# purejade/pinot

Measured on AMD Instinct MI355X. Metric: rows/sec for filter+group-by SUM at 1/2/4/8 GPUs; % of HBM roofline, higher is better.
Workload: dtype int64; 1 GPU; c5: BASELINE configs[4]: 4096 x 2M rows sharded over the GPUs, (f1 IN 32 ids OR f2=7) AND f3<>3, group by gk (card 1000), sum(m); segments=4096, rows_total=8192000000, parallelism=dp1 (segment sharding)

## Files before the change

### pinot_amd/csrc/pgx_host.cpp

```cpp
#include "pgx_host.h"


namespace pgxh {
size_t align_up(size_t x, size_t a) { return (x + a - 1) & ~(a - 1); }

void canon_rprog(std::vector<int>& op, std::vector<int>& arg) {
  struct Node { int op, arg, l, r; };
  std::vector<Node> nodes;
  std::vector<int> st;
  for (size_t i = 0; i < op.size(); ++i) {
    Node nd{op[i], arg[i], -1, -1};
    if (op[i] == RP_NOT) {
      if (st.empty()) return;
      nd.l = st.back();
      st.pop_back();
    } else if (op[i] != RP_LEAF) {
      if (st.size() < 2) return;
      nd.r = st.back();
      st.pop_back();
      nd.l = st.back();
      st.pop_back();
    }
    nodes.push_back(nd);
    st.push_back(int(nodes.size()) - 1);
// ... 545 lines not shown
      J.narrow_vbits = P.part_narrow ? P.narrow_vd : 0;
      J.narrow_unit = P.kn.narrow_unit;
      J.prefetch2 = P.part_narrow && P.kn.prefetch2;
    }
    J.dense_slots = P.dense_slots;
    if ((K.group_mode == G_DENSE_LDS || K.group_mode == G_HASH64 || K.group_mode == G_HASH128) &&
        K.num_planes == 2 && K.num_aggs == 1 && (K.agg_kind[0] == A_SUM || K.agg_kind[0] == A_AVG) && !P.use_part) {
      const int c = K.agg_col[0];
      if (c >= 0 && J.cols[c].img != IMG_NONE && !J.cols[c].fp) {
        int64_t maxdocs = 1, ntiles = 0;
        uint64_t vrange = 0;
        const int64_t trows = int64_t(J.T) * J.TL;
        for (int sg : members) {
          maxdocs = std::max<int64_t>(maxdocs, P.ksegs[sg].num_docs);
          vrange = std::max<uint64_t>(vrange, P.segcols[sg][c]->vrange);
          ntiles += (int64_t(P.ksegs[sg].num_docs) + trows - 1) / trows;
        }
        maxdocs = std::min<int64_t>(maxdocs, (ntiles + cus - 1) / cus * trows);
        const int cb = bits_for(maxdocs + 1);
        const long double sum_max = (long double)maxdocs * (long double)(vrange + 1);
        int sb = 0;
        while (sb < 64 && std::ldexp(1.0L, sb) <= sum_max) ++sb;
        if (cb + sb <= 64) J.dense_pack = 64 - cb;
      }
    }
    if (hp1 && !J.dense_pack && hashg) {
      hp1 = false;
      while (hash_slots > 512 && lds_need() > lds_budget) hash_slots /= 2;
      J.hash_slots = hash_slots;
    }
    J.leafmask = P.fsm_on && P.lmask_off[members[0]] >= 0;
    J.compact = P.rchunk && !P.use_part;
    J.selmask = P.want_selmask;

    ExecPlan::JitGroup G;
    G.T = J.T;
    int lds_bytes = 0;
    std::string err;
    G.fn = jit_function(J, ctx->device, &lds_bytes, &err);
    if (!G.fn) fail(PGX_ERR_INTERNAL, "query kernel compile: " + err);
    const int64_t tile_rows = int64_t(J.T) * J.TL;
    int64_t tiles = 0;
    for (int s : members) {
      const KSeg& S = P.ksegs[s];
      JSeg js{};
      js.tile_begin = tiles;
      js.num_docs = S.num_docs;
      js.rec_base = P.rec_base[s];
      js.lmask = S.lmask;
      js.lmask_words = S.lmask_words;
      js.selmask = P.want_selmask ? P.sel_buf.as<unsigned int>() + P.sel_off[s] : nullptr;
      if (P.star[s].on) {
        auto& tl = P.star_tiles[s];
        tl.clear();
        for (const auto& r : P.star[s].ranges)
          for (int k = 0; k < r.second; ++k) {
            const int32_t a = P.blob32[r.first + 2 * k], b = P.blob32[r.first + 2 * k + 1];
            for (int64_t t = a / tile_rows; t <= b / tile_rows; ++t)
              if (tl.empty() || tl.back() != int32_t(t)) tl.push_back(int32_t(t));
          }
        std::sort(tl.begin(), tl.end());
        tl.erase(std::unique(tl.begin(), tl.end()), tl.end());
        const size_t off = star_tile_off;
        star_tile_off += tl.size();
        if (star_tile_off > P.star_tile_cap) fail(PGX_ERR_INTERNAL, "star tile list overflow");
        std::memcpy(B.host.bytes() + B.off_tiles + off * 4, tl.data(), tl.size() * 4);
// ... 1543 lines not shown
```

### pinot_amd/csrc/pgx_internal.h

```cpp
#pragma once
#include <stdint.h>

#include "pgx_jit_abi.h"

namespace pgx {

constexpr int kTileRows = 8192;
constexpr int kLaneRows = 32;
constexpr int kBlock = 256;
constexpr int kMaxQCols = 16;
constexpr int kMaxLeaves = 64;
constexpr int kInlineLeaves = PGX_J_MAX_LEAVES;
constexpr int kMaxLeafSlots = PGX_J_MAX_SLOTS;
constexpr int kStarMaxLeaves = 8;
constexpr int kMaxAggs = 8;
constexpr int kMaxGroupCols = 16;
constexpr int kMaxProg = 192;
constexpr int kStackDepth = 8;
constexpr uint64_t kEmptyKey = ~0ull;

enum LeafMode : int8_t {
  LEAF_SCAN_INTERVAL = 0,
  LEAF_SCAN_BITSET = 1,
  LEAF_RANGES = 2,
// ... 327 lines not shown
#include <vector>

namespace pgx {

enum ImgKind : int8_t {
  IMG_NONE = 0,
  IMG_U32 = 1,
  IMG_FOR16 = 2,
  IMG_F64 = 3,
};
constexpr int kImgFor16Blocks = 64;
constexpr int kLdsBudget = 160 * 1024 - 256;

constexpr uint64_t kNarrowC1 = 0x9E3779B1ull;
constexpr int kNarrow1Bits = 8;
constexpr int kNarrowRing = 64;
constexpr int kNarrowMaxBits2 = 10;
enum RProgKind { RPROG_AUTO = -1, RPROG_OFF = 0, RPROG_WAVE = 1, RPROG_SEG = 2, RPROG_CHUNK = 3, RPROG_STACK = 4 };
struct Knobs {
  bool jit = true;
  bool narrow = true;
  bool narrow_direct = false;
  bool narrow_gather = false;
  int rchunk = -1;
  int rprog = RPROG_AUTO;
  int batch_segs = -1;
  bool no_img = false;
  bool prefetch2 = false;
  int narrow_unit = 32;
  int lone_head = 2;
  bool part_small = false;
  int narrow_k2 = -1;
  bool narrow_log = false;
  bool host_profile = false;
};
Knobs read_knobs();

struct NarrowMix {
  uint64_t mask = 0, c1 = kNarrowC1, ic1 = 0;
  int s = 0;
};
inline uint64_t narrow_inverse(uint64_t c) {
  uint64_t x = c;
  for (int i = 0; i < 6; ++i) x *= 2 - c * x;
  return x;
}
inline NarrowMix narrow_mix(int keybits) {
  NarrowMix m;
  m.mask = keybits >= 64 ? ~0ull : (uint64_t(1) << keybits) - 1u;
  m.s = (keybits + 1) / 2;
  m.ic1 = narrow_inverse(m.c1);
  return m;
}

struct JitCol {
  int bits = 0;
  bool decode = false;
  int img = IMG_NONE;
  int img_sh = 0;
  int img_words = 0;
  bool acc32 = false;
  bool fp = false;
  bool remap = false;
  bool frac = false;
};

struct JitShape {
  int T = 256;
  int R = 8;
  int TL = 32;
  std::vector<JitCol> cols;
  std::vector<int> leaf_col, leaf_mode;
  std::vector<int> prog_op, prog_arg;
  std::vector<int> agg_kind, agg_col, plane_op;
  int group_mode = G_NONE;
  std::vector<int> gcol;
  std::vector<uint64_t> gmul;
  uint64_t dense_slots = 0;
  int num_planes = 1;
  std::vector<int> gshift;
  int keybits = 0;
  int emit_col = -1;
  std::vector<int> ghi;
  int hash_slots = 0;
  bool leafmask = false;
  std::vector<std::vector<int>> rprog_ops;
  int part_bits = 0;
  bool emit_dictid = false;
  bool part_slab = false;
  int dense_pack = 0;
  bool compact = false;
  bool selmask = false;
  bool part_narrow = false;
  int narrow_vbits = 0;
  int narrow_unit = 32;
  bool prefetch2 = false;
};

constexpr int kFsmMaxLeaves = 10;
constexpr int kFsmMaxStates = 4096;
constexpr uint64_t kFsmMaxTable = 1ull << 22;
constexpr int kFsmChunkRows = 1024;
constexpr int kFsmMaxIntervals = 3 * kFsmMaxLeaves + 2;

struct FsmTreeNode {
  int op = 0;
  int leaf = -1;
  int phys = 3;
  std::vector<FsmTreeNode> kids;
};
struct FsmSegInfo {
  int32_t num_docs = 0;
  std::vector<int64_t> sorted_first, sorted_last;
  uint32_t always_false = 0;
};
struct FsmPlan {
  int num_states = 0, num_leaves = 0, num_tables = 0;
  std::vector<uint32_t> table;
  std::vector<std::vector<std::pair<int32_t, int32_t>>> seg_intervals;
};
bool fsm_build(const FsmTreeNode& tree, int num_leaves, const std::vector<FsmSegInfo>& segs, FsmPlan& out,
               std::string* err);

std::string jit_source(const JitShape& s, int* lds_bytes);
void* jit_function(const JitShape& s, int device, int* lds_bytes, std::string* err);

}
```

### pinot_amd/csrc/pgx_jit.cpp

```cpp
#include <hip/hip_runtime.h>
#include <hip/hiprtc.h>
#include <sys/stat.h>
#include <unistd.h>

#include <algorithm>
#include <cstdio>
#include <cstdlib>
#include <map>
#include <mutex>
#include <sstream>
#include <string>
#include <vector>

#include "pgx_internal.h"

extern "C" int pgx_jit_compile_check(const char* source, char* log, unsigned long log_cap);

namespace pgx {

namespace {

const char* kAbiSrc =
#include "pgx_jit_abi.inc"
    ;
// ... 340 lines not shown
      }
    if (grouped)
      for (size_t g = 0; g < s.gcol.size(); ++g)
        if (s.cols[s.gcol[g]].remap) gremap[g] = split = true;
  }
  const bool pack = s.dense_pack > 0 && s.group_mode == G_DENSE_LDS && s.num_planes == 2 && naggs == 1 &&
                    (s.agg_kind[0] == A_SUM || s.agg_kind[0] == A_AVG) && !s.cols[s.agg_col[0]].fp &&
                    s.cols[s.agg_col[0]].img != IMG_NONE && !emit;
  for (int c = 0; c < ncols; ++c) {
    if (need_vb[c]) e.ln("const i64 vb", c, " = S->vbase[", c, "];");
    if (need_dict[c]) {
      if (s.cols[c].fp) e.ln("const PGX_G double* __restrict__ dd", c, " = (const PGX_G double*)S->dict[", c, "];");
      else e.ln("const PGX_G i64* __restrict__ di", c, " = (const PGX_G i64*)S->dict[", c, "];");
    }
  }
  if (scr_off >= 0) e.ln("int rc_cur = -1;  // chunk whose bitmap-program masks are in LDS");
  e.ln("u64 wcnt = 0;  // selected rows of this wave in this segment (wave-uniform)");
  if (!grouped) {
    for (int a = 0; a < naggs; ++a) {
      const int k = s.agg_kind[a];
      const int c = s.agg_col[a];
      if (k == A_SUM || k == A_AVG) {
        if (s.cols[c].fp) e.ln("double acc", a, " = 0.0;");
        else if (s.cols[c].img == IMG_NONE) e.ln("i64 acc", a, " = 0;");
        else e.ln("u64 acc", a, " = 0;");
      } else if (k == A_MIN) {
        e.ln("u32 mn", a, " = 0xFFFFFFFFu;");
      } else if (k == A_MAX) {
        e.ln("u32 mx", a, " = 0u;");
      }
    }
  }
  int gate = -1;
  {
    bool all_masks = !s.prog_op.empty();
    for (size_t pc = 0; pc < s.prog_op.size() && all_masks; ++pc)
      if (s.prog_op[pc] == OP_LEAF && !is_docmask(s.leaf_mode[s.prog_arg[pc]])) all_masks = false;
    std::vector<std::vector<int>> impl;
    for (size_t pc = 0; pc < s.prog_op.size() && all_masks; ++pc) {
      const int op = s.prog_op[pc], arg = s.prog_arg[pc];
      if (op == OP_LEAF) {
        impl.push_back(s.leaf_mode[arg] == LEAF_DOCMASK ? std::vector<int>{arg} : std::vector<int>{});
      } else if (op == OP_AND || op == OP_OR) {
        std::vector<int> acc = impl.back();
        impl.pop_back();
        for (int k = 1; k < arg; ++k) {
          std::vector<int> x = impl.back(), y;
          impl.pop_back();
          if (op == OP_AND) {
            y = acc;
            y.insert(y.end(), x.begin(), x.end());
          } else {
            for (int l : acc)
              if (std::find(x.begin(), x.end(), l) != x.end()) y.push_back(l);
          }
          acc = y;
        }
        impl.push_back(acc);
      } else if (op == OP_TRUE) {
        impl.push_back({});
      }
    }
    if (all_masks && impl.size() == 1 && !impl[0].empty() && !compact) gate = impl[0][0];
  }
  auto gate_bits = [&](const std::string& w) {
    return s.R == 32 ? w : "((" + w + " >> (r0 & 31)) & " + std::to_string((1u << s.R) - 1u) + "u)";
  };
  auto emit_loads = [&](const std::string& tile, const std::string& dst, const std::string& rbv = "rbn") {
    e.ln("{");
    e.ind++;
    e.ln(rbv, " = (int)((tl ? (long long)tl[", tile, " - tile0] : (", tile, " - tile0)) * (PT * PTL));");
    e.ln("const int rb = ", rbv, ";");
    e.ln("const bool full = rb + PT * PTL <= nd;");
    for (int u = 0; u < U; ++u) {
      e.ln("{");
      e.ind++;
      e.ln("const int r0 = rb + ", u * s.R, " * PT + tid * PR;");
      const std::string cond =
          gate >= 0 ? "(full || r0 < nd) && " + gate_bits("ga[" + std::to_string(u) + "]") + " != 0u" : "full || r0 < nd";
      for (int c = 0; c < ncols; ++c) {
        if (!s.cols[c].decode) continue;
        const int D = dwords_per(s, c);
        if (s.cols[c].frac)
          e.ln("if (", cond, ") pgx_ld_u<", D, ">(f", c, " + (((long long)r0 * ", s.cols[c].bits, ") >> 5), &", dst,
               c, "[", u * D, "]); else pgx_zero<", D, ">(&", dst, c, "[", u * D, "]);");
        else
        e.ln("if (", cond, ") pgx_ld<", D, ">(f", c, " + (long long)(r0 / PR) * ", D, ", &", dst, c, "[", u * D,
             "]); else pgx_zero<", D, ">(&", dst, c, "[", u * D, "]);");
      }
      for (int l = 0; l < nleaves; ++l)
        if (l == gate) e.ln(dst, "q", l, "[", u, "] = ga[", u, "];");
        else if (is_docmask(s.leaf_mode[l]))
          e.ln(dst, "q", l, "[", u, "] = (full || r0 < nd) ? dm", l, "[r0 >> 5] : 0u;");
      e.ind--;
      e.ln("}");
    }
// ... 100 lines not shown
        e.ln("    const u32 keep = dw >= nd ? 0u : (dw + 32 > nd ? (1u << (nd - dw)) - 1u : 0xFFFFFFFFu);");
      }
      std::vector<std::string> st;
      int leaf = 0, tmp = 0;
      for (int op : ops) {
        const std::string X = "y" + std::to_string(tmp++);
        if (op == RP_LEAF) {
          e.ln("    const u32 ", X, " = rlm", l, "[", leaf++ * 2048, " + w];");
        } else if (op == RP_NOT) {
          e.ln("    const u32 ", X, " = ~", st.back(), " & keep;");
          st.pop_back();
        } else {
          const std::string b = st.back();
          st.pop_back();
          const std::string a = st.back();
          st.pop_back();
          e.ln("    const u32 ", X, " = ", a, op == RP_AND ? " & " : " | ", b, ";");
        }
        st.push_back(X);
      }
      e.ln("    rlm", l, "[w] = ", st.empty() ? std::string("0u") : st.back(), ";");
      e.ln("  }");
    }
    e.ln("  pgx_lds_barrier();");
    e.ln("}");
  }
  e.ln("auto body = [&](auto FT) {");
  e.ind = 4;
  e.ln("constexpr bool FULL = decltype(FT)::value;");
  for (int u = 0; u < U; ++u) {
    e.ln("{");
    e.ind = 5;
    e.ln("const int r0 = rb + ", u * s.R, " * PT + tid * PR;");
    for (int c = 0; c < ncols; ++c) {
      if (!s.cols[c].decode) continue;
      e.ln("u32 v", c, "[PR];");
      if (s.cols[c].frac)
        e.ln("pgx_unpack_frac<", s.cols[c].bits, ", PR, ", dwords_per(s, c), ">(&c", c, "[", u * dwords_per(s, c),
             "], (u32)(((long long)r0 * ", s.cols[c].bits, ") & 31), v", c, ");");
      else
        e.ln("pgx_unpack<", s.cols[c].bits, ", PR>(&c", c, "[", u * dwords_per(s, c), "], v", c, ");");
    }
    for (int l = 0; l < nleaves; ++l) {
      if (s.leaf_mode[l] == LEAF_RANGES) e.ln("const u32 W", l, " = pgx_ranges_bits(rg", l, ", nr", l, ", cur", l, ", r0, PR);");
      if (is_docmask(s.leaf_mode[l])) e.ln("const u32 W", l, " = cq", l, "[", u, "] >> (r0 & 31);");
      if (s.leaf_mode[l] == LEAF_RCHUNK) e.ln("const u32 W", l, " = rlm", l, "[(r0 & 0xFFFF) >> 5] >> (r0 & 31);");
    }
    if (!grouped)
      for (int a = 0; a < naggs; ++a) {
        const int k = s.agg_kind[a];
        if ((k == A_SUM || k == A_AVG) && !s.cols[s.agg_col[a]].fp && s.cols[s.agg_col[a]].img != IMG_NONE &&
            s.cols[s.agg_col[a]].acc32)
          e.ln("u32 p", a, " = 0u;");
      }
    if (emit) e.ln("u64 recs[PR];");
    if (split) e.ln("u32 msk = 0u;");
    if (s.selmask) e.ln("u32 smk = 0u;");
    if (s.leafmask)
      for (int l = 0; l < nleaves; ++l) e.ln("u32 lw", l, " = 0u;");
    e.ln("#pragma unroll");
    e.ln("for (int j = 0; j < PR; ++j) {");
    e.ind = 6;
    e.ln("const bool vj = FULL || (r0 + j < nd);");
    std::vector<std::string> st;
    int tmp = 0;
    for (size_t pc = 0; pc < s.prog_op.size(); ++pc) {
      const int op = s.prog_op[pc], arg = s.prog_arg[pc];
      if (op == OP_LEAF) {
        const int l = arg, c = s.leaf_col[l];
        const std::string B = "b" + std::to_string(tmp++);
        const std::string v = "v" + std::to_string(c) + "[j]";
        switch (s.leaf_mode[l]) {
          case LEAF_SCAN_INTERVAL:
            e.ln("const bool ", B, " = vj && ((", v, " - lo", l, ") <= sp", l, ");");
            break;
          case LEAF_SCAN_BITSET:
            e.ln("const bool ", B, " = vj && ((bs", l, "[", v, " >> 5] >> (", v, " & 31u)) & 1u);");
            break;
          case LEAF_RANGES:
          case LEAF_DOCMASK:
          case LEAF_RCHUNK:
            e.ln("const bool ", B, " = vj && ((W", l, " >> j) & 1u);");
            break;
          case LEAF_DOCMASK_NOT:
            e.ln("const bool ", B, " = vj && !((W", l, " >> j) & 1u);");
            break;
          default:
// ... 155 lines not shown
          encs[a] = "ev" + std::to_string(a);
        }
      if (hpack) {
        const int c = s.agg_col[0];
        e.ln("const u64 hv = (1ull << ", s.dense_pack, ") + (u64)", img_value(s, c, img_off, "v" + std::to_string(c) + "[j]"),
             ";");
      }
      e.ln("const int ls = ", h128 ? "pgx_lhash128(hk, hst, " + std::to_string(HS) + ", klo, khi)"
                                   : "pgx_lhash64(hk, " + std::to_string(HS) + ", klo)", ";");
      e.ln("if (ls >= 0) {");
      if (hpack) {
        e.ln("  atomicAdd(&ht[ls], hv);");
      } else {
        e.ln("  atomicAdd(&ht[ls], 1ull);");
        for (int a = 0; a < naggs; ++a)
          if (s.agg_kind[a] != A_COUNT)
            e.ln("  ", plane_atomic(s.plane_op[a + 1], "&ht[" + std::to_string((a + 1) * HS) + " + ls]", encs[a]));
      }
      e.ln("} else {");
      e.ln("  const long long gs = ", h128 ? "pgx_ghash128((PGX_G unsigned long long*)A.hkeys, (PGX_G unsigned int*)A.hstate, A.hash_cap, klo, khi, A.overflow)"
                                           : "pgx_ghash64((PGX_G unsigned long long*)A.hkeys, A.hash_cap, klo, A.overflow)", ";");
      e.ln("  if (gs < 0) {");
      e.ln("    atomicAdd(A.overflow, 1ull);");
      e.ln("  } else {");
      e.ln("    atomicAdd(A.table + gs, 1ull);");
      for (int a = 0; a < naggs; ++a)
        if (s.agg_kind[a] != A_COUNT)
          e.ln("    ", plane_atomic(s.plane_op[a + 1], "A.table + " + std::to_string(a + 1) + " * A.hash_cap + gs", encs[a]));
      e.ln("  }");
      e.ln("}");
      e.ind = 6;
      e.ln("}");
    };
    if (!grouped) {
      for (int a = 0; a < naggs; ++a) {
        const int k = s.agg_kind[a];
        if (k == A_COUNT) continue;
        const int c = s.agg_col[a];
        const JitCol& C = s.cols[c];
        const std::string v = "v" + std::to_string(c) + "[j]";
        if (k == A_MIN) {
          e.ln("mn", a, " = min(mn", a, ", m ? ", v, " : 0xFFFFFFFFu);");
        } else if (k == A_MAX) {
          e.ln("mx", a, " = max(mx", a, ", m ? ", v, " : 0u);");
        } else if (C.fp) {
          const std::string val = (C.img == IMG_F64)
                                      ? "((const double*)lds)[" + std::to_string(img_off[c] / 8) + " + " + v + "]"
                                      : (gcolv[c] ? "gv" + std::to_string(c) + "[j]" : "dd" + std::to_string(c) + "[" + v + "]");
          e.ln("if (m) acc", a, " += ", val, ";");
        } else if (C.img == IMG_NONE) {
          if (gcolv[c]) e.ln("acc", a, " += gv", c, "[j];");
          else e.ln("if (m) acc", a, " += di", c, "[", v, "];");
        } else if (C.acc32) {
          e.ln("{ const u32 x = ", img_value(s, c, img_off, v), "; p", a, " += m ? x : 0u; }");
        } else {
          e.ln("{ const u32 x = ", img_value(s, c, img_off, v), "; acc", a, " += m ? (u64)x : 0ull; }");
        }
      }
    } else {
      if (emit) {
        e.ln("u64 rec = ~0ull;");
        e.ln("if (m) {");
        std::string key = "0ull";
        for (size_t g = 0; g < s.gcol.size(); ++g) {
          const int c = s.gcol[g];
          std::string id = "v" + std::to_string(c) + "[j]";
          if (s.cols[c].remap) id = "(u32)rm" + std::to_string(g) + "[" + id + "]";
          key += " | ((u64)" + id + " << " + std::to_string(s.gshift[g]) + ")";
        }
        std::string x = "0u";
        if (s.emit_col >= 0) {
          const std::string ec = std::to_string(s.emit_col);
          if (s.emit_dictid) x = "(u32)(v" + ec + "[j] + (u32)S->emit_rebase)";
          else x = s.cols[s.emit_col].img != IMG_NONE
                       ? "(u32)(" + img_value(s, s.emit_col, img_off, "v" + ec + "[j]") + " + (u32)S->emit_rebase)"
                       : "(u32)(di" + ec + "[v" + ec + "[j]] - S->vbase[" + ec + "] + S->emit_rebase)";
        }
        if (enarrow) {
          const NarrowMix mx = narrow_mix(s.keybits);
          const std::string M = std::to_string(mx.mask) + "ull";
          e.ln("  u64 h = ((", key, ") * ", mx.c1, "ull) & ", M, ";");
          e.ln("  h ^= h >> ", mx.s, ";");
          e.ln("  rec = ((h >> ", nrb1, ") << 56) | (h & ", (uint64_t(1) << nrb1) - 1u, "ull) | ((u64)(", x, ") << ", nrb1,
               ");");
        } else {
          e.ln("  rec = (", key, ") | ((u64)(", x, ") << ", s.keybits, ");");
        }
        e.ln("}");
        e.ln("recs[j] = rec;");
      } else if (hashm) {
        emit_hash();
      } else {
        emit_dense();
      }
    }
    e.ind = 5;
    e.ln("}");
    if (compact) {
      e.ln("  pgx_wave_lds_sync();");
      e.ln("}");
    }
    if (!grouped)
      for (int a = 0; a < naggs; ++a) {
        const int k = s.agg_kind[a];
        if ((k == A_SUM || k == A_AVG) && !s.cols[s.agg_col[a]].fp && s.cols[s.agg_col[a]].img != IMG_NONE &&
            s.cols[s.agg_col[a]].acc32)
          e.ln("acc", a, " += p", a, ";");
      }
    if (s.selmask) {
      const char* ty = s.R == 8 ? "unsigned char" : (s.R == 16 ? "unsigned short" : "unsigned int");
      e.ln("if (FULL || r0 < nd) ((PGX_G ", ty, "*)S->selmask)[r0 / PR] = (", ty, ")smk;");
    }
    if (s.leafmask) {
      const char* ty = s.R == 8 ? "unsigned char" : (s.R == 16 ? "unsigned short" : "unsigned int");
      e.ln("if (FULL || r0 < nd) {");
      for (int l = 0; l < nleaves; ++l)
        e.ln("  ((PGX_G ", ty, "*)(S->lmask + ", l, " * S->lmask_words))[r0 / PR] = (", ty, ")lw", l, ";");
      e.ln("}");
    }
    if (enarrow) {
      const std::string NR = std::to_string(NRG), NUs = std::to_string(NU);
      e.ln("{");
      e.ln("  u32 pp[PR];");
      e.ln("  #pragma unroll");
      e.ln("  for (int j = 0; j < PR; ++j) pp[j] = recs[j] != ~0ull ? atomicAdd(&ncur[(u32)(recs[j] >> 56)], 1u) : 0u;");
      e.ln("  pgx_lds_barrier();");
      e.ln("  const u32* const Ucur = nU + npar * 256;");
      e.ln("  const u32* const Vcur = nV + npar * 256;");
      e.ln("  if (tid < 256) {");
      e.ln("    const u32 en = ncur[tid], u0 = Ucur[tid], v0 = Vcur[tid];");
      e.ln("    const u32 lim = u0 + ", NR, "u;");
      e.ln("    const u32 nu = (((en < lim) ? en : lim) - u0) / ", NUs, "u;");
// ... 249 lines not shown
  int lds = 0;
};

std::mutex g_jit_mu;
std::map<std::pair<int, std::string>, JitEntry> g_jit_cache;

}

std::vector<int64_t> shape_key(const JitShape& s, int device) {
  std::vector<int64_t> k{device, s.T, s.R, s.TL, s.group_mode, int64_t(s.dense_slots), s.num_planes, s.keybits, s.emit_col,
                         int64_t(s.cols.size()), s.leafmask};
  for (const JitCol& c : s.cols)
    k.insert(k.end(), {c.bits, c.decode, c.img, c.img_sh, c.img_words, c.acc32, c.fp, c.remap, c.frac});
  auto add = [&](const auto& v) {
    k.push_back(-int64_t(v.size()) - 1);
    for (auto x : v) k.push_back(int64_t(x));
  };
  add(s.leaf_col);
  add(s.leaf_mode);
  add(s.prog_op);
  add(s.prog_arg);
  add(s.agg_kind);
  add(s.agg_col);
  add(s.plane_op);
  add(s.gcol);
  add(s.gmul);
  add(s.gshift);
  for (const auto& ops : s.rprog_ops) add(ops);
  k.push_back(s.part_bits);
  k.push_back(s.emit_dictid);
  k.push_back(s.part_slab);
  k.push_back(s.dense_pack);
  k.push_back(s.compact);
  k.push_back(s.selmask);
  k.push_back(s.part_narrow);
  k.push_back(s.narrow_vbits);
  k.push_back(s.narrow_unit);
  k.push_back(s.prefetch2);
  add(s.ghi);
  k.push_back(s.hash_slots);
  return k;
}

std::map<std::vector<int64_t>, JitEntry> g_jit_shapes;

constexpr const char* kJitOpts[] = {"--offload-arch=gfx950", "-O3", "-std=c++17"};

std::string jit_cache_dir() {
  const char* d = std::getenv("PGX_JIT_CACHE");
  return d && *d ? d : "";
}

uint64_t text_hash(const std::string& t, uint64_t h, uint64_t mul) {
  for (unsigned char c : t) {
    h ^= c;
    h *= mul;
  }
  return h;
}

std::string cache_text(const std::string& src) {
  std::string t = src;
  for (const char* o : kJitOpts) t += std::string("\n//") + o;
  return t;
}

// ... 77 lines not shown
      if (err) *err = "hiprtcCreateProgram failed";
      return nullptr;
    }
    const hiprtcResult rc = hiprtcCompileProgram(prog, 3, const_cast<const char**>(pgx::kJitOpts));
    if (rc != HIPRTC_SUCCESS) {
      size_t n = 0;
      hiprtcGetProgramLogSize(prog, &n);
      std::string log(n, '\0');
      if (n) hiprtcGetProgramLog(prog, &log[0]);
      hiprtcDestroyProgram(&prog);
      if (err) *err = "hiprtc compile failed: " + log.substr(0, 4000);
      return nullptr;
    }
    size_t code_size = 0;
    hiprtcGetCodeSize(prog, &code_size);
    code.assign(code_size, '\0');
    hiprtcGetCode(prog, &code[0]);
    hiprtcDestroyProgram(&prog);
    cache_store(src, code);
  }
  JitEntry ent;
  ent.lds = lds;
  if (hipModuleLoadData(&ent.mod, code.data()) != hipSuccess ||
      hipModuleGetFunction(&ent.fn, ent.mod, "pgxq") != hipSuccess) {
    if (err) *err = "hipModuleLoadData / hipModuleGetFunction failed";
    return nullptr;
  }
  g_jit_cache.emplace(key, ent);
  g_jit_shapes.emplace(skey, ent);
  return ent.fn;
}

}

extern "C" int pgx_jit_compile_check(const char* source, char* log, unsigned long log_cap) {
  hiprtcProgram prog;
  if (hiprtcCreateProgram(&prog, source, "pgx_query.hip", 0, nullptr, nullptr) != HIPRTC_SUCCESS) return -1;
  const hiprtcResult rc = hiprtcCompileProgram(prog, 3, const_cast<const char**>(pgx::kJitOpts));
  size_t n = 0;
  hiprtcGetProgramLogSize(prog, &n);
  if (log && log_cap) {
    std::string l(n, '\0');
    if (n) hiprtcGetProgramLog(prog, &l[0]);
    std::snprintf(log, log_cap, "%s", l.c_str());
  }
  if (rc == HIPRTC_SUCCESS)
    if (const char* dir = std::getenv("PGX_JIT_DUMP")) {
      size_t cs = 0;
      hiprtcGetCodeSize(prog, &cs);
      std::string code(cs, '\0');
      hiprtcGetCode(prog, &code[0]);
      if (FILE* f = std::fopen((std::string(dir) + "/last_check.co").c_str(), "wb")) {
        std::fwrite(code.data(), 1, cs, f);
        std::fclose(f);
      }
    }
  hiprtcDestroyProgram(&prog);
  return rc == HIPRTC_SUCCESS ? 0 : 1;
}

extern "C" int pgx_jit_selftest(int* n_total, char* log, unsigned long log_cap) {
  using namespace pgx;
  std::vector<JitShape> shapes;
  auto base = [](int bits_f, int bits_m, int img, int sh) {
    JitShape s;
    s.cols.resize(2);
// ... 125 lines not shown
    s.agg_col = {-1, 1, 1, 1, 1};
    s.plane_op = {P_ADD_I64, P_ADD_I64, P_ADD_I64, P_MIN_ORD, P_MAX_ORD, P_ADD_I64};
    s.num_planes = 6;
    shapes.push_back(s);
    s.cols[1].img = IMG_U32;
    s.cols[1].img_words = 1024;
    shapes.push_back(s);
    s.compact = false;
    s.selmask = true;
    shapes.push_back(s);
  }
  {
    JitShape s = base(10, 16, IMG_FOR16, 11);
    s.cols[1].img_words = 64 + 32768;
    s.cols.push_back(JitCol{});
    s.cols[2].bits = 10;
    s.cols[2].decode = false;
    s.leaf_col = {2, 2, 2, -1};
    s.leaf_mode = {LEAF_NONE, LEAF_NONE, LEAF_NONE, LEAF_DOCMASK};
    s.prog_op = {OP_LEAF, OP_STAT};
    s.prog_arg = {3, 0};
    s.R = 16;
    s.T = 1024;
    s.group_mode = G_DENSE_LDS;
    s.gcol = {0};
    s.gmul = {1};
    s.dense_slots = 1000;
    s.agg_kind = {A_SUM};
    s.agg_col = {1};
    s.plane_op = {P_ADD_I64, P_ADD_I64};
    s.num_planes = 2;
    s.dense_pack = 40;
    shapes.push_back(s);
  }
  for (int R : {8, 16, 32}) {
    JitShape s = base(R == 8 ? 8 : (R == 16 ? 10 : 7), 16, IMG_FOR16, 11);
    s.cols.push_back(JitCol{});
    s.cols[2].bits = 4;
    s.leaf_col = {0, 2, 0};
    s.leaf_mode = {LEAF_SCAN_INTERVAL, LEAF_RANGES, LEAF_DOCMASK_NOT};
    s.prog_op = {OP_LEAF, OP_LEAF, OP_LEAF, OP_OR, OP_AND};
    s.prog_arg = {0, 1, 2, 2, 2};
    s.R = R;
    s.leafmask = true;
    shapes.push_back(s);
  }
  {
    JitShape s = base(14, 16, IMG_FOR16, 11);
    s.cols.push_back(JitCol{});
    s.cols[2].bits = 20;
    s.cols[2].decode = true;
    s.leaf_col.clear();
    s.leaf_mode.clear();
    s.prog_op.clear();
    s.prog_arg.clear();
    s.R = 16;
    s.T = 512;
    s.group_mode = G_EMIT;
    s.gcol = {0, 2};
    s.gshift = {0, 14};
    s.keybits = 34;
    s.emit_col = 1;
    s.agg_kind = {A_SUM, A_MIN, A_MAX};
    s.agg_col = {1, 1, 1};
    s.plane_op = {P_ADD_I64, P_ADD_I64, P_MIN_ORD, P_MAX_ORD};
    s.num_planes = 4;
// ... 211 lines not shown
```

### pinot_amd/csrc/pgx_jit_device.h

```cpp
template <int D>
__device__ __forceinline__ void pgx_ld(const u32* __restrict__ gp, u32* w) {
  const PGX_G u32* p = (const PGX_G u32*)gp;
  if constexpr (D % 4 == 0) {
#pragma unroll
    for (int i = 0; i < D / 4; ++i) {
      pgx_u32x4 q = __builtin_nontemporal_load((const PGX_G pgx_u32x4*)p + i);
      w[4 * i] = q.x; w[4 * i + 1] = q.y; w[4 * i + 2] = q.z; w[4 * i + 3] = q.w;
    }
  } else if constexpr (D % 2 == 0) {
#pragma unroll
    for (int i = 0; i < D / 2; ++i) {
      pgx_u32x2 q = __builtin_nontemporal_load((const PGX_G pgx_u32x2*)p + i);
      w[2 * i] = q.x; w[2 * i + 1] = q.y;
    }
  } else {
#pragma unroll
    for (int i = 0; i < D; ++i) w[i] = __builtin_nontemporal_load(p + i);
  }
}

template <int D>
__device__ __forceinline__ void pgx_ld_u(const u32* __restrict__ gp, u32* w) {
  const PGX_G u32* p = (const PGX_G u32*)gp;
#pragma unroll
// ... 48 lines not shown
    for (int i = 0; i < D; ++i) w[i] = __builtin_bswap32(raw[i]);
    w[D] = 0u;
    constexpr u32 MASK = (1u << B) - 1u;
#pragma unroll
    for (int j = 0; j < R; ++j) {
      const int o = j * B;
      const int k = o >> 5;
      const int s = o & 31;
      if (s + B <= 32) v[j] = (w[k] >> (32 - s - B)) & MASK;
      else v[j] = __builtin_amdgcn_alignbit(w[k], w[k + 1], 64 - s - B) & MASK;
    }
  }
}

template <int B, int R, int DL>
__device__ __forceinline__ void pgx_unpack_frac(const u32* raw, u32 sh, u32* v) {
  u32 w[DL];
#pragma unroll
  for (int i = 0; i < DL; ++i) w[i] = __builtin_bswap32(raw[i]);
  constexpr int D = (R * B + 31) / 32;
  u32 x[D + 1];
#pragma unroll
  for (int i = 0; i < D; ++i) x[i] = sh ? __builtin_amdgcn_alignbit(w[i], i + 1 < DL ? w[i + 1] : 0u, 32u - sh) : w[i];
  x[D] = 0u;
  constexpr u32 MASK = (1u << B) - 1u;
#pragma unroll
  for (int j = 0; j < R; ++j) {
    const int o = j * B;
    const int k = o >> 5;
    const int s = o & 31;
    if (s + B <= 32) v[j] = (x[k] >> (32 - s - B)) & MASK;
    else v[j] = __builtin_amdgcn_alignbit(x[k], x[k + 1], 64 - s - B) & MASK;
  }
}

__device__ __forceinline__ u32 pgx_valid_bits(int r0, int nd, int R) {
  if (r0 >= nd) return 0u;
  const int n = nd - r0;
  if (n >= R) return (R == 32) ? 0xFFFFFFFFu : ((1u << R) - 1u);
  return (1u << n) - 1u;
}

__device__ __forceinline__ u32 pgx_ranges_bits(const PGX_G int* __restrict__ r, int nr, int& cur, int r0, int R) {
  while (cur < nr && r[2 * cur + 1] < r0) ++cur;
  u32 word = 0u;
  const int last = r0 + R - 1;
  for (int i = cur; i < nr; ++i) {
    const int a = r[2 * i], b = r[2 * i + 1];
    if (a > last) break;
    const int s = max(a, r0) - r0, e = min(b, last) - r0;
    word |= (e - s == 31) ? 0xFFFFFFFFu : (((1u << (e - s + 1)) - 1u) << s);
  }
  return word;
}

__device__ __forceinline__ int pgx_ranges_seek(const PGX_G int* __restrict__ r, int nr, int r0) {
  int lo = 0, hi = nr;
  while (lo < hi) {
    const int mid = (lo + hi) >> 1;
    if (r[2 * mid + 1] < r0) lo = mid + 1; else hi = mid;
  }
  return lo;
}

__device__ __forceinline__ u64 pgx_wsum_u64(u64 x) {
#pragma unroll
// ... 92 lines not shown
```

### pinot_amd/csrc/pgx_plan.cpp

```cpp
#include <cstring>
#include "pgx_host.h"

namespace pgxh {

PNode build_tree(const pgx_query& q, const pgx_segment& seg0) {
  std::vector<PNode> st;
  for (const auto& n : q.filter) {
    if (n.op == PGX_F_LEAF) {
      if (n.arg < 0 || n.arg >= int(q.leaf_col.size())) fail(PGX_ERR_INVALID_ARG, "filter leaf index out of range");
      PNode p;
      p.op = PGX_F_LEAF;
      p.leaf = n.arg;
      const StagedColumn& c = seg0.col(q.leaf_col[n.arg]);
      if (c.has_inverted && q.leaf_kind[n.arg] != PGX_PRED_RANGE) p.phys = c.is_sorted ? PH_SORTED : PH_BITMAP;
      else p.phys = PH_SCAN;
      st.push_back(std::move(p));
    } else if (n.op == PGX_F_AND || n.op == PGX_F_OR) {
      if (n.arg < 1 || n.arg > int(st.size())) fail(PGX_ERR_INVALID_ARG, "filter node arity");
      PNode p;
      p.op = n.op;
      p.phys = n.op == PGX_F_AND ? PH_AND : PH_OR;
      p.kids.assign(std::make_move_iterator(st.end() - n.arg), std::make_move_iterator(st.end()));
      st.erase(st.end() - n.arg, st.end());
      std::stable_sort(p.kids.begin(), p.kids.end(), [](const PNode& a, const PNode& b) { return a.phys < b.phys; });
// ... 214 lines not shown
}

Knobs pgx::read_knobs() {
  Knobs k;
  auto env = [](const char* name) -> std::string {
    const char* e = std::getenv(name);
    return e ? std::string(e) : std::string();
  };
  const std::string jit = env("PGX_JIT"), nar = env("PGX_PART_NARROW"), rc = env("PGX_RCHUNK"), rp = env("PGX_RPROG");
  const std::string bs = env("PGX_BATCH_SEGS"), dbg = env("PGX_DEBUG");
  k.jit = !(jit.size() && jit[0] == '0');
  k.narrow = !(nar.size() && nar[0] == '0');
  k.narrow_direct = nar == "direct";
  k.narrow_gather = nar == "gather";
  if (rc.size()) k.rchunk = rc[0] == '1' ? 1 : 0;
  if (rp == "off") k.rprog = RPROG_OFF;
  else if (rp == "wave") k.rprog = RPROG_WAVE;
  else if (rp == "seg") k.rprog = RPROG_SEG;
  else if (rp == "chunk") k.rprog = RPROG_CHUNK;
  else if (rp == "stack") k.rprog = RPROG_STACK;
  if (bs.size()) k.batch_segs = std::atoi(bs.c_str());
  size_t i = 0;
  while (i < dbg.size()) {
    size_t j = dbg.find(',', i);
    if (j == std::string::npos) j = dbg.size();
    const std::string o = dbg.substr(i, j - i);
    if (o == "part_small") k.part_small = true;
    else if (o == "narrow_log") k.narrow_log = true;
    else if (o == "host_profile") k.host_profile = true;
    else if (o.rfind("narrow_k2=", 0) == 0) k.narrow_k2 = std::atoi(o.c_str() + 10);
    else if (o == "nunit=16") k.narrow_unit = 16;
    else if (o == "pf2") k.prefetch2 = true;
    else if (o == "noimg") k.no_img = true;
    else if (o.rfind("head=", 0) == 0) k.lone_head = std::max(2, std::atoi(o.c_str() + 5));
    i = j + 1;
  }
  return k;
}

namespace pgxh {

int qslot(ExecPlan& P, const std::string& name) {
  for (size_t i = 0; i < P.qcols.size(); ++i)
    if (P.qcols[i] == name) return int(i);
  if (P.qcols.size() >= size_t(kMaxQCols)) fail(PGX_ERR_UNSUPPORTED, "query touches too many columns");
  P.qcols.push_back(name);
  return int(P.qcols.size() - 1);
}

bool star_fit(const pgx_query& q, const pgx_segment& seg) {
  if (!seg.st_ok || (q.flags & PGX_Q_NO_STAR_TREE) || q.agg_fn.empty()) return false;
  auto skipped = [&](const std::string& c) {
    return std::find(seg.st_skip.begin(), seg.st_skip.end(), c) != seg.st_skip.end();
  };
  for (const auto& g : q.group_cols)
    if (skipped(g)) return false;
  for (const auto& c : q.leaf_col)
    if (skipped(c)) return false;
  for (int fn : q.agg_fn)
    if (fn != PGX_SUM) return false;
  const size_t nl = q.leaf_col.size();
  if (!q.filter.empty()) {
    if (q.filter.size() == 1) {
      if (q.filter[0].op != PGX_F_LEAF) return false;
    } else {
      if (q.filter.back().op != PGX_F_AND || q.filter.back().arg != int(nl) || q.filter.size() != nl + 1) return false;
// ... 1293 lines not shown
```

Baseline: 1457 billion rows/s.

## Add sparse row-iteration path for mask-only filters in JIT kernel

When the filter is built entirely from docmask leaves, the generated kernel now computes the selection word first. It only does the full per-row unpack and dense update if some lane has more than sparse_k selected rows. Otherwise it loops over the set bits and extracts single fields with new pgx_unpack_at helpers. This is meant to avoid decoding every row's group and value columns when selectivity is low, at the cost of a divergent per-bit loop and extra select-tree code when rows are moderately dense. Debug knobs densebody and sparsek=N are added, along with a unit check kernel.

New measurement: 1497 billion rows/s, median of 6. 2.7% higher.

```diff
diff --git a/pinot_amd/csrc/pgx_host.cpp b/pinot_amd/csrc/pgx_host.cpp
--- a/pinot_amd/csrc/pgx_host.cpp
+++ b/pinot_amd/csrc/pgx_host.cpp
@@ -601,6 +601,8 @@
     J.leafmask = P.fsm_on && P.lmask_off[members[0]] >= 0;
     J.compact = P.rchunk && !P.use_part;
     J.selmask = P.want_selmask;
+    J.dense_body = P.kn.dense_body;
+    if (P.kn.sparse_k >= 0) J.sparse_k = P.kn.sparse_k;
 
     ExecPlan::JitGroup G;
     G.T = J.T;
diff --git a/pinot_amd/csrc/pgx_internal.h b/pinot_amd/csrc/pgx_internal.h
--- a/pinot_amd/csrc/pgx_internal.h
+++ b/pinot_amd/csrc/pgx_internal.h
@@ -383,6 +383,8 @@
   bool part_small = false;
   int narrow_k2 = -1;
   bool narrow_log = false;
+  bool dense_body = false;
+  int sparse_k = -1;
   bool host_profile = false;
 };
 Knobs read_knobs();
@@ -403,6 +405,8 @@
   m.ic1 = narrow_inverse(m.c1);
   return m;
 }
+
+constexpr int kSparseK = 4;
 
 struct JitCol {
   int bits = 0;
@@ -446,6 +450,8 @@
   int narrow_vbits = 0;
   int narrow_unit = 32;
   bool prefetch2 = false;
+  bool dense_body = false;
+  int sparse_k = kSparseK;
 };
 
 constexpr int kFsmMaxLeaves = 10;
diff --git a/pinot_amd/csrc/pgx_jit.cpp b/pinot_amd/csrc/pgx_jit.cpp
--- a/pinot_amd/csrc/pgx_jit.cpp
+++ b/pinot_amd/csrc/pgx_jit.cpp
@@ -396,6 +396,7 @@
     }
   }
   int gate = -1;
+  bool sparse = false;
   {
     bool all_masks = !s.prog_op.empty();
     for (size_t pc = 0; pc < s.prog_op.size() && all_masks; ++pc)
@@ -426,6 +427,13 @@
       }
     }
     if (all_masks && impl.size() == 1 && !impl[0].empty() && !compact) gate = impl[0][0];
+    bool has_leaf = false, stat_tail = true;
+    for (size_t pc = 0; pc < s.prog_op.size(); ++pc) {
+      has_leaf |= s.prog_op[pc] == OP_LEAF;
+      if (pc && s.prog_op[pc - 1] == OP_STAT && s.prog_op[pc] != OP_STAT) stat_tail = false;
+    }
+    sparse = all_masks && has_leaf && stat_tail && impl.size() == 1 && !s.dense_body && !emit && !hashm && !compact &&
+             !s.selmask && !s.leafmask;
   }
   auto gate_bits = [&](const std::string& w) {
     return s.R == 32 ? w : "((" + w + " >> (r0 & 31)) & " + std::to_string((1u << s.R) - 1u) + "u)";
@@ -592,15 +600,18 @@
     e.ln("{");
     e.ind = 5;
     e.ln("const int r0 = rb + ", u * s.R, " * PT + tid * PR;");
-    for (int c = 0; c < ncols; ++c) {
-      if (!s.cols[c].decode) continue;
-      e.ln("u32 v", c, "[PR];");
-      if (s.cols[c].frac)
-        e.ln("pgx_unpack_frac<", s.cols[c].bits, ", PR, ", dwords_per(s, c), ">(&c", c, "[", u * dwords_per(s, c),
-             "], (u32)(((long long)r0 * ", s.cols[c].bits, ") & 31), v", c, ");");
-      else
-        e.ln("pgx_unpack<", s.cols[c].bits, ", PR>(&c", c, "[", u * dwords_per(s, c), "], v", c, ");");
-    }
+    auto emit_unpack = [&]() {
+      for (int c = 0; c < ncols; ++c) {
+        if (!s.cols[c].decode) continue;
+        e.ln("u32 v", c, "[PR];");
+        if (s.cols[c].frac)
+          e.ln("pgx_unpack_frac<", s.cols[c].bits, ", PR, ", dwords_per(s, c), ">(&c", c, "[", u * dwords_per(s, c),
+               "], (u32)(((long long)r0 * ", s.cols[c].bits, ") & 31), v", c, ");");
+        else
+          e.ln("pgx_unpack<", s.cols[c].bits, ", PR>(&c", c, "[", u * dwords_per(s, c), "], v", c, ");");
+      }
+    };
+    if (!sparse) emit_unpack();
     for (int l = 0; l < nleaves; ++l) {
       if (s.leaf_mode[l] == LEAF_RANGES) e.ln("const u32 W", l, " = pgx_ranges_bits(rg", l, ", nr", l, ", cur", l, ", r0, PR);");
       if (is_docmask(s.leaf_mode[l])) e.ln("const u32 W", l, " = cq", l, "[", u, "] >> (r0 & 31);");
@@ -613,6 +624,32 @@
             s.cols[s.agg_col[a]].acc32)
           e.ln("u32 p", a, " = 0u;");
       }
+    if (sparse) {
+      std::vector<std::string> ws;
+      int tmp = 0;
+      for (size_t pc = 0; pc < s.prog_op.size(); ++pc) {
+        const int op = s.prog_op[pc], arg = s.prog_arg[pc];
+        if (op == OP_LEAF) {
+          ws.push_back(std::string(s.leaf_mode[arg] == LEAF_DOCMASK_NOT ? "~W" : "W") + std::to_string(arg));
+        } else if (op == OP_AND || op == OP_OR) {
+          for (int k = 1; k < arg; ++k) {
+            const std::string b = ws.back();
+            ws.pop_back();
+            const std::string a = ws.back();
+            ws.pop_back();
+            const std::string X = "sw" + std::to_string(tmp++);
+            e.ln("const u32 ", X, " = ", a, op == OP_AND ? " & " : " | ", b, ";");
+            ws.push_back(X);
+          }
+        } else if (op == OP_TRUE) {
+          ws.push_back("0xFFFFFFFFu");
+        }
+      }
+      e.ln("u32 sel = ", ws.back(), s.R == 32 ? std::string() : " & " + std::to_string((1u << s.R) - 1u) + "u", ";");
+      e.ln("if (!FULL) sel &= pgx_valid_bits(r0, nd, PR);");
+      e.ln("if (__ballot(__popc(sel) > ", s.sparse_k, ") != 0ull) {");
+      emit_unpack();
+    }
     if (emit) e.ln("u64 recs[PR];");
     if (split) e.ln("u32 msk = 0u;");
     if (s.selmask) e.ln("u32 smk = 0u;");
@@ -834,6 +871,7 @@
       e.ind = 6;
       e.ln("}");
     };
+    auto emit_update = [&]() {
     if (!grouped) {
       for (int a = 0; a < naggs; ++a) {
         const int k = s.agg_kind[a];
@@ -896,10 +934,52 @@
         emit_dense();
       }
     }
+    };
+    emit_update();
     e.ind = 5;
     e.ln("}");
     if (compact) {
       e.ln("  pgx_wave_lds_sync();");
+      e.ln("}");
+    }
+    if (sparse) {
+      bool stat = false;
+      for (int op : s.prog_op) stat |= op == OP_STAT;
+      e.ln("} else {");
+      e.ind = 6;
+      e.ln("for (;;) {");
+      e.ind = 7;
+      e.ln("const bool m = sel != 0u;");
+      e.ln("const unsigned long long sb = __ballot(m);");
+      e.ln("if (sb == 0ull) break;");
+      e.ln("wcnt += __popcll(sb);");
+      if (stat) e.ln("st_ent += __popcll(sb);");
+      e.ln("const u32 sj = m ? (u32)__builtin_ctz(sel) : 0u;");
+      e.ln("sel &= sel - 1u;");
+      e.ln("const int j = 0;");
+      std::vector<bool> need(ncols, false);
+      if (grouped)
+        for (int c : s.gcol) need[c] = true;
+      for (int a = 0; a < naggs; ++a)
+        if (s.agg_kind[a] != A_COUNT) need[s.agg_col[a]] = true;
+      for (int c = 0; c < ncols; ++c) {
+        if (!need[c]) continue;
+        const int D = dwords_per(s, c);
+        if (s.cols[c].frac)
+          e.ln("const u32 v", c, "[1] = {pgx_unpack_frac_at<", s.cols[c].bits, ", PR, ", D, ">(&c", c, "[", u * D,
+               "], (u32)(((long long)r0 * ", s.cols[c].bits, ") & 31), sj)};");
+        else
+          e.ln("const u32 v", c, "[1] = {pgx_unpack_at<", s.cols[c].bits, ", PR>(&c", c, "[", u * D, "], sj)};");
+      }
+      for (int c = 0; c < ncols; ++c)
+        if (gcolv[c]) e.ln(s.cols[c].fp ? "double" : "i64", " gv", c, "[1] = {m ? ", s.cols[c].fp ? "dd" : "di", c,
+                           "[v", c, "[0]] : 0};");
+      for (size_t g = 0; g < s.gcol.size(); ++g)
+        if (gremap[g]) e.ln("u32 gr", g, "[1] = {m ? (u32)rm", g, "[v", s.gcol[g], "[0]] : 0u};");
+      emit_update();
+      e.ind = 6;
+      e.ln("}");
+      e.ind = 5;
       e.ln("}");
     }
     if (!grouped)
@@ -1215,6 +1295,8 @@
   k.push_back(s.part_slab);
   k.push_back(s.dense_pack);
   k.push_back(s.compact);
+  k.push_back(s.dense_body);
+  k.push_back(s.sparse_k);
   k.push_back(s.selmask);
   k.push_back(s.part_narrow);
   k.push_back(s.narrow_vbits);
@@ -1358,6 +1440,8 @@
 }
 
 }
+
+extern "C" int pgx_sparse_k() { return pgx::kSparseK; }
 
 extern "C" int pgx_jit_compile_check(const char* source, char* log, unsigned long log_cap) {
   hiprtcProgram prog;
@@ -1549,6 +1633,45 @@
     s.num_planes = 2;
     s.dense_pack = 40;
     shapes.push_back(s);
+    s.dense_body = true;
+    shapes.push_back(s);
+    s.dense_body = false;
+    s.dense_pack = 0;
+    s.leaf_col = {2, -1};
+    s.leaf_mode = {LEAF_DOCMASK_NOT, LEAF_DOCMASK};
+    s.prog_op = {OP_LEAF, OP_LEAF, OP_AND, OP_STAT};
+    s.prog_arg = {1, 0, 2, 0};
+    s.cols[2].decode = true;
+    s.cols[2].bits = 4;
+    s.gcol = {0, 2};
+    s.gmul = {1, 1000};
+    s.dense_slots = 8000;
+    s.group_mode = G_DENSE_GLOBAL;
+    s.agg_kind = {A_COUNT, A_SUM, A_MIN, A_MAX};
+    s.agg_col = {-1, 1, 1, 1};
+    s.plane_op = {P_ADD_I64, P_ADD_I64, P_ADD_I64, P_MIN_ORD, P_MAX_ORD};
+    s.num_planes = 5;
+    shapes.push_back(s);
+    s.group_mode = G_NONE;
+    s.gcol.clear();
+    s.gmul.clear();
+    s.cols[2].bits = 7;
+    s.cols[2].img = IMG_NONE;
+    s.leaf_col = {2};
+    s.leaf_mode = {LEAF_DOCMASK_NOT};
+    s.prog_op = {OP_LEAF};
+    s.prog_arg = {0};
+    s.agg_kind = {A_COUNT, A_SUM, A_MIN, A_MAX, A_AVG, A_MAX};
+    s.agg_col = {-1, 1, 1, 1, 1, 2};
+    s.plane_op = {P_ADD_I64, P_ADD_I64, P_ADD_I64, P_MIN_ORD, P_MAX_ORD, P_ADD_I64, P_MAX_ORD};
+    s.num_planes = 7;
+    s.R = 32;
+    s.T = 512;
+    shapes.push_back(s);
+    s.R = 8;
+    s.TL = 16;
+    s.cols[0].frac = s.cols[2].frac = true;
+    shapes.push_back(s);
   }
   for (int R : {8, 16, 32}) {
     JitShape s = base(R == 8 ? 8 : (R == 16 ? 10 : 7), 16, IMG_FOR16, 11);
diff --git a/pinot_amd/csrc/pgx_jit_device.h b/pinot_amd/csrc/pgx_jit_device.h
--- a/pinot_amd/csrc/pgx_jit_device.h
+++ b/pinot_amd/csrc/pgx_jit_device.h
@@ -104,6 +104,57 @@
     if (s + B <= 32) v[j] = (x[k] >> (32 - s - B)) & MASK;
     else v[j] = __builtin_amdgcn_alignbit(x[k], x[k + 1], 64 - s - B) & MASK;
   }
+}
+
+template <int LO, int LEVEL, int D>
+__device__ __forceinline__ u32 pgx_pick(const u32* raw, u32 k) {
+  if constexpr (LEVEL == 0) {
+    return raw[LO];
+  } else {
+    constexpr int H = 1 << (LEVEL - 1);
+    const u32 a = pgx_pick<LO, LEVEL - 1, D>(raw, k);
+    if constexpr (LO + H >= D) {
+      return a;
+    } else {
+      const u32 b = pgx_pick<LO + H, LEVEL - 1, D>(raw, k);
+      return (k & (u32)H) ? b : a;
+    }
+  }
+}
+template <int D>
+__device__ __forceinline__ u32 pgx_pick_dword(const u32* raw, u32 k) {
+  constexpr int LV = D <= 1 ? 0 : (D <= 2 ? 1 : (D <= 4 ? 2 : (D <= 8 ? 3 : (D <= 16 ? 4 : (D <= 32 ? 5 : 6)))));
+  return pgx_pick<0, LV, D>(raw, k);
+}
+template <int B, int D>
+__device__ __forceinline__ u32 pgx_field_at(const u32* raw, u32 o) {
+  constexpr u32 MASK = B == 32 ? 0xFFFFFFFFu : ((1u << (B & 31)) - 1u);
+  const u32 e = o + (u32)(B - 1);
+  const u32 k = e >> 5;
+  const u32 lo = __builtin_bswap32(pgx_pick_dword<D>(raw, k));
+  const u32 n = 31u - (e & 31u);
+  if constexpr (32 % B == 0) {
+    return (lo >> n) & MASK;
+  } else {
+    const u32 hi = __builtin_bswap32(pgx_pick_dword<D>(raw, k - 1u));
+    return __builtin_amdgcn_alignbit(hi, lo, n) & MASK;
+  }
+}
+template <int B, int R>
+__device__ __forceinline__ u32 pgx_unpack_at(const u32* raw, u32 j) {
+  if constexpr (B == 16)
+    return __builtin_amdgcn_perm(0u, pgx_pick_dword<R / 2>(raw, j >> 1), (j & 1u) ? 0x0c0c0203u : 0x0c0c0001u);
+  else
+    return pgx_field_at<B, R * B / 32>(raw, j * (u32)B);
+}
+template <int B, int R, int DL>
+__device__ __forceinline__ u32 pgx_unpack_frac_at(const u32* raw, u32 sh, u32 j) {
+  constexpr u32 MASK = B == 32 ? 0xFFFFFFFFu : ((1u << (B & 31)) - 1u);
+  const u32 e = sh + j * (u32)B + (u32)(B - 1);
+  const u32 k = e >> 5;
+  const u32 lo = __builtin_bswap32(pgx_pick_dword<DL>(raw, k));
+  const u32 hi = __builtin_bswap32(pgx_pick_dword<DL>(raw, k - 1u));
+  return __builtin_amdgcn_alignbit(hi, lo, 31u - (e & 31u)) & MASK;
 }
 
 __device__ __forceinline__ u32 pgx_valid_bits(int r0, int nd, int R) {
diff --git a/pinot_amd/csrc/pgx_plan.cpp b/pinot_amd/csrc/pgx_plan.cpp
--- a/pinot_amd/csrc/pgx_plan.cpp
+++ b/pinot_amd/csrc/pgx_plan.cpp
@@ -270,6 +270,8 @@
     else if (o == "nunit=16") k.narrow_unit = 16;
     else if (o == "pf2") k.prefetch2 = true;
     else if (o == "noimg") k.no_img = true;
+    else if (o == "densebody") k.dense_body = true;
+    else if (o.rfind("sparsek=", 0) == 0) k.sparse_k = std::min(32, std::max(0, std::atoi(o.c_str() + 8)));
     else if (o.rfind("head=", 0) == 0) k.lone_head = std::max(2, std::atoi(o.c_str() + 5));
     i = j + 1;
   }
diff --git a/pinot_amd/csrc/pgx_unpack_check.hip b/pinot_amd/csrc/pgx_unpack_check.hip
--- /dev/null
+++ b/pinot_amd/csrc/pgx_unpack_check.hip
@@ -0,0 +1,76 @@
+#include <hip/hip_runtime.h>
+#include <stdint.h>
+
+#include "pgx_jit_abi.h"
+#include "pgx_device.h"
+#include "pgx_jit_device.h"
+
+namespace {
+
+template <int B, int R, bool FRAC>
+__global__ void pgx_unpack_at_check(const u32* __restrict__ fwd, int n, const u32* __restrict__ js, u32* at, u32* ref) {
+  const int i = blockIdx.x * blockDim.x + threadIdx.x;
+  if (i >= n) return;
+  u32 v[R];
+  if constexpr (FRAC) {
+    constexpr int RB = R * B;
+    constexpr int G = RB % 32 == 0 ? 32 : (RB % 16 == 0 ? 16 : (RB % 8 == 0 ? 8 : (RB % 4 == 0 ? 4 : (RB % 2 == 0 ? 2 : 1))));
+    constexpr int DL = (RB + 32 - G + 31) / 32;
+    const long long o = (long long)i * RB;
+    const u32 sh = (u32)(o & 31);
+    u32 w[DL];
+#pragma unroll
+    for (int k = 0; k < DL; ++k) w[k] = fwd[(o >> 5) + k];
+    pgx_unpack_frac<B, R, DL>(w, sh, v);
+#pragma unroll
+    for (int q = 0; q < R; ++q) ref[(long long)i * R + q] = v[q];
+#pragma unroll 1
+    for (int q = 0; q < R; ++q) at[(long long)i * R + q] = pgx_unpack_frac_at<B, R, DL>(w, sh, js[q]);
+  } else {
+    constexpr int D = R * B / 32;
+    u32 w[D];
+#pragma unroll
+    for (int k = 0; k < D; ++k) w[k] = fwd[(long long)i * D + k];
+    pgx_unpack<B, R>(w, v);
+#pragma unroll
+    for (int q = 0; q < R; ++q) ref[(long long)i * R + q] = v[q];
+#pragma unroll 1
+    for (int q = 0; q < R; ++q) at[(long long)i * R + q] = pgx_unpack_at<B, R>(w, js[q]);
+  }
+}
+
+template <int B, int R>
+hipError_t launch_br(bool frac, const u32* fwd, int n, const u32* js, u32* at, u32* ref, hipStream_t st) {
+  const dim3 grid((n + 255) / 256), block(256);
+  if (frac) {
+    if constexpr (B == 32) return hipErrorInvalidValue;
+    else hipLaunchKernelGGL((pgx_unpack_at_check<B, R, true>), grid, block, 0, st, fwd, n, js, at, ref);
+  } else {
+    if constexpr ((R * B) % 32 != 0) return hipErrorInvalidValue;
+    else hipLaunchKernelGGL((pgx_unpack_at_check<B, R, false>), grid, block, 0, st, fwd, n, js, at, ref);
+  }
+  return hipGetLastError();
+}
+
+template <int B>
+hipError_t launch_b(int R, bool frac, const u32* fwd, int n, const u32* js, u32* at, u32* ref, hipStream_t st) {
+  if (R == 8) return launch_br<B, 8>(frac, fwd, n, js, at, ref, st);
+  if (R == 16) return launch_br<B, 16>(frac, fwd, n, js, at, ref, st);
+  if (R == 32) return launch_br<B, 32>(frac, fwd, n, js, at, ref, st);
+  return hipErrorInvalidValue;
+}
+
+template <int B>
+hipError_t launch_from(int bits, int R, bool frac, const u32* fwd, int n, const u32* js, u32* at, u32* ref, hipStream_t st) {
+  if (bits == B) return launch_b<B>(R, frac, fwd, n, js, at, ref, st);
+  if constexpr (B < 32) return launch_from<B + 1>(bits, R, frac, fwd, n, js, at, ref, st);
+  else return hipErrorInvalidValue;
+}
+
+}
+
+extern "C" hipError_t pgx_launch_unpack_at_check(int bits, int R, int frac, const uint32_t* fwd, int n, const uint32_t* js,
+                                                 uint32_t* at, uint32_t* ref, hipStream_t stream) {
+  if (bits < 1 || bits > 32 || n < 1 || !fwd || !js || !at || !ref) return hipErrorInvalidValue;
+  return launch_from<1>(bits, R, frac != 0, fwd, n, js, at, ref, stream);
+}
```
